# tensorflow/recommenders

Measured on AMD Instinct MI355X. Metric: queries/sec brute-force top-100, higher is better.
Workload: dtype f32; 1 GPU; BruteForce top-100, 1M-item x dim-64 corpus, batch 8192 (BASELINE.json configs[1]); corpus_rows_total=1000000, corpus_rows_per_gpu=1000000, dim=64, batch=8192, k=100, parallelism=single GPU

## Files before the change

include/tfrs_hip.h:

```cpp
#ifndef TFRS_HIP_H_
#define TFRS_HIP_H_

#include <stddef.h>
#include <stdint.h>

#ifdef __cplusplus
extern "C" {
#endif

#define TFRS_OK 0
#define TFRS_EINVAL (-1)
#define TFRS_ENOTIMPL (-2)
#define TFRS_EHIP (-3)
#define TFRS_ENOMEM (-4)
#define TFRS_ESTATE (-5)

#define TFRS_MAX_DIM 128
#define TFRS_MAX_K 1024

int tfrs_version(void);
const char *tfrs_last_error(void);
int tfrs_device_info(int dev, int *cu_count_h, int *lds_bytes_h, char *arch_h,
                     int arch_len);
int tfrs_set_option(const char *name, const char *value);
// ... 37 lines not shown
size_t tfrs_bruteforce_topk_below_workspace_bytes(int64_t nq, int64_t n, int d, int k);
int tfrs_bruteforce_topk_below(const tfrs_index_t *index, const float *queries, int64_t nq, int k,
                               const float *last_scores, const int32_t *last_rows, int64_t last_ld,
                               float *out_scores, int32_t *out_idx, void *workspace,
                               size_t workspace_bytes, void *stream);
int tfrs_bruteforce_topk_redo_count(const void *workspace, int64_t nq, int64_t n, int k,
                                    int32_t *redo_count_h, void *stream);
int tfrs_bruteforce_topk_redo_reasons(const void *workspace, int64_t nq, int64_t n, int k,
                                      int32_t *reasons_h, void *stream);

int tfrs_debug_topk_plan(int64_t n, int k, int shuffled, int64_t *plan_h);

int tfrs_debug_fp16_scores(const tfrs_index_t *index, const float *queries, int64_t nq,
                           int64_t row_begin, int64_t row_end, float *out, float *scratch,
                           void *stream);

size_t tfrs_streaming_topk_workspace_bytes(int64_t nq, int64_t nb, int d, int k);
int tfrs_streaming_topk_update(const float *queries, int64_t nq, int d,
                               const float *cand_block, int64_t nb, int64_t base_row,
                               int k, float *state_scores, int32_t *state_idx,
                               int32_t state_len, int32_t *new_len_h, void *workspace,
                               size_t workspace_bytes, void *stream);

size_t tfrs_streaming_topk_blocks_workspace_bytes(int64_t nq, int64_t total_rows, int d, int k);
int tfrs_streaming_topk_update_blocks(const float *queries, int64_t nq, int d,
                                      const float *const *blocks_h, const int64_t *block_rows_h,
                                      int nblocks, int64_t base_row, int64_t seen_rows, int k,
                                      float *state_scores, int32_t *state_idx, int32_t state_len,
                                      int32_t *new_len_h, void *workspace, size_t workspace_bytes,
                                      void *stream);
// ... 306 lines not shown
```

recommenders_amd/_lib.py:

```python

import ctypes
import os
from typing import Optional

_PKG = os.path.dirname(os.path.abspath(__file__))
LIB_PATH = os.path.join(_PKG, "libtfrs_hip.so")

TFRS_OK, TFRS_EINVAL, TFRS_ENOTIMPL, TFRS_EHIP, TFRS_ENOMEM, TFRS_ESTATE = 0, -1, -2, -3, -4, -5

c_void_p, c_int, c_i64, c_size_t, c_float = (ctypes.c_void_p, ctypes.c_int, ctypes.c_int64,
                                             ctypes.c_size_t, ctypes.c_float)
P = c_void_p
c_u64 = ctypes.c_uint64

SIGNATURES = {
    "tfrs_version": (c_int, []),
    "tfrs_last_error": (ctypes.c_char_p, []),
    "tfrs_device_info": (c_int, [c_int, P, P, P, c_int]),
    "tfrs_set_option": (c_int, [ctypes.c_char_p, ctypes.c_char_p]),
    "tfrs_get_option": (c_int, [ctypes.c_char_p, ctypes.c_char_p, c_int]),
    "tfrs_profile_enable": (c_int, [c_int]),
    "tfrs_profile_read": (c_int, [P, P, P]),
    "tfrs_profile_read_kind": (c_int, [c_int, P, P, P]),
    "tfrs_calibrate_workspace_bytes": (c_size_t, []),
# ... 7 lines not shown
    "tfrs_index_nonfinite": (c_int, [P, c_int, P]),
    "tfrs_index_note_nonfinite": (c_int, [P, P, c_i64, P, c_i64, c_int, P]),
    "tfrs_index_size": (c_i64, [P]),
    "tfrs_index_dim": (c_int, [P]),
    "tfrs_index_unpack": (c_int, [P, P, P]),
    "tfrs_bruteforce_topk_workspace_bytes": (c_size_t, [c_i64, c_i64, c_int, c_int]),
    "tfrs_bruteforce_topk": (c_int, [P, P, c_i64, c_int, P, P, P, c_size_t, P]),
    "tfrs_row_hash64": (c_int, [P, c_i64, c_int, P, P]),
    "tfrs_topk_expand_duplicates": (c_int, [P, P, c_i64, c_int, P, P, c_int, P, P, P]),
    "tfrs_bruteforce_topk_below_workspace_bytes": (c_size_t, [c_i64, c_i64, c_int, c_int]),
    "tfrs_bruteforce_topk_below": (c_int, [P, P, c_i64, c_int, P, P, c_i64, P, P, P, c_size_t, P]),
    "tfrs_bruteforce_topk_redo_count": (c_int, [P, c_i64, c_i64, c_int, P, P]),
    "tfrs_bruteforce_topk_redo_reasons": (c_int, [P, c_i64, c_i64, c_int, P, P]),
    "tfrs_debug_topk_plan": (c_int, [c_i64, c_int, c_int, P]),
    "tfrs_debug_fp16_scores": (c_int, [P, P, c_i64, c_i64, c_i64, P, P, P]),
    "tfrs_streaming_topk_workspace_bytes": (c_size_t, [c_i64, c_i64, c_int, c_int]),
    "tfrs_streaming_topk_update": (c_int, [P, c_i64, c_int, P, c_i64, c_i64, c_int, P, P,
                                           ctypes.c_int32, P, P, c_size_t, P]),
    "tfrs_streaming_topk_blocks_workspace_bytes": (c_size_t, [c_i64, c_i64, c_int, c_int]),
    "tfrs_streaming_topk_update_blocks": (c_int, [P, c_i64, c_int, P, P, c_int, c_i64, c_i64, c_int, P, P,
                                                  ctypes.c_int32, P, P, c_size_t, P]),
    "tfrs_compute_scores": (c_int, [P, P, c_i64, c_int, c_int, P, c_int, P, c_size_t, P]),
    "tfrs_topk_update_from_scores": (c_int, [P, c_i64, c_i64, c_i64, c_i64, c_int, P, P, ctypes.c_int32,
                                             P, P]),
    "tfrs_topk_merge_workspace_bytes": (c_size_t, [c_i64, c_int, c_int, c_int]),
    "tfrs_topk_merge": (c_int, [P, P, c_int, c_i64, c_int, c_int, P, P, P, c_size_t, P]),
    "tfrs_topk_merge_strided": (c_int, [P, P, c_int, c_i64, c_i64, c_int, c_int, P, P, P]),
    "tfrs_topk_exclude": (c_int, [P, P, c_i64, c_int, P, c_int, c_int, P, P, P]),
    "tfrs_rank_of_positive": (c_int, [P, P, c_i64, c_int, P, c_int, P, c_int, P, P]),
    "tfrs_id_match_topk": (c_int, [P, P, c_i64, c_int, P, c_int, P, P]),
# ... 171 lines not shown
```

recommenders_amd/csrc/common.h:

```cpp
#pragma once

#include <hip/hip_runtime.h>
#include <stdint.h>
#include <stdio.h>

#include "../../include/tfrs_hip.h"

namespace tfrs {

void set_error(const char *fmt, ...);

#define TFRS_CHECK_ARG(cond, ...)        \
  do {                                   \
    if (!(cond)) {                       \
      ::tfrs::set_error(__VA_ARGS__);    \
      return TFRS_EINVAL;                \
    }                                    \
  } while (0)

#define TFRS_HIP(call)                                                        \
  do {                                                                        \
    hipError_t e_ = (call);                                                   \
    if (e_ != hipSuccess) {                                                   \
      ::tfrs::set_error("%s failed: %s (%s:%d)", #call, hipGetErrorString(e_), \
// ... 205 lines not shown
  int64_t row_limit;
  int n_qtiles;
  int n_splits;
  const float *lower;
  const float *qk;
  const float *qscale;
  uint32_t *cnt;
  uint2 *buf;
  uint32_t cap_l;
  int nseg;
  float *dense;
  int64_t ld_dense;
  float *binmax;
  int64_t ld_binmax;
  int bin_stages;
  uint32_t *ovf_cnt;
  uint2 *ovf_buf;
  uint32_t ovf_cap;
  int drain_every;
  int drain_min;
  uint32_t *zero_aux;
  uint32_t *zero_word;
};
int launch_scan16(const Scan16Args &a, hipStream_t stream);
constexpr int kScan16QueriesPerWg = 512;

enum SelectSource { kSrcDense = 0, kSrcList = 1, kSrcParts = 2, kSrcRecompute = 3, kSrcExpand = 4 };

struct SelectArgs {
  int64_t nq;
  int k;
  const float *state_scores;
  const int32_t *state_idx;
  int state_len;
  int source;
  const float *dense;
  int64_t ld_dense;
  int64_t n_dense;
  const uint2 *buf;
// ... 61 lines not shown
```

recommenders_amd/csrc/topk_api.hip:

```cpp
#include <stdlib.h>

#include <algorithm>
#include <new>

#include "common.h"

namespace tfrs {

static int64_t env_i64(const char *name, int64_t dflt) {
  const char *v = option(name);
  if (!v || !*v) return dflt;
  return atoll(v);
}

struct TopkTuning {
  int64_t prefix;
  int64_t rho;
  int64_t target_wgs;
  int64_t thr_wgs;
  bool f16_filter;
  int64_t sample;
  int64_t min_bins;
  int64_t drain_min;
  int64_t drain_every;
// ... 392 lines not shown
  se.k = k;
  se.q = q;
  se.d = d;
  se.source = kSrcRecompute;
  se.only_flagged = w.redo;
  se.part_keys = w.part_keys;
  se.idx_base = idx_base;
  se.rc_begin = row_lo;
  se.rc_end = row_lo + n;
  se.raw = raw;
  se.out_scores = out_scores;
  se.out_idx = out_idx;
  return launch_recompute(se, stream);
}

static int run_f16(const float *q, int64_t nq, int d, const char *packed, const F16Image &img,
                   int64_t n, int64_t idx_base, int k, const SamplePlan &sp, bool lower_preset,
                   float *out_scores, int32_t *out_idx, const RoundWs &w, const TopkTuning &t,
                   hipStream_t stream, const int32_t *rowmap = nullptr, int64_t row_lo = 0,
                   const RawTable *raw = nullptr, uint32_t *flags = nullptr) {
  const int n_qtiles = (int)((nq + kScan16QueriesPerWg - 1) / kScan16QueriesPerWg);
  const int64_t stage_lo = row_lo / kTileN;
  int rc;
  if ((rc = launch_query_kappa(q, nq, d, w.qk, w.qscale, w.ovf_cnt, stream, flags)) != TFRS_OK) return rc;

  Scan16Args s16 = {};
  s16.q = q;
  s16.nq = nq;
  s16.d = d;
  s16.packed16 = img.packed16;
  s16.meta = img.meta;
  s16.n_qtiles = n_qtiles;
  s16.qk = w.qk;
  s16.qscale = w.qscale;
  s16.row_limit = row_lo + n;
  s16.stage0 = stage_lo;

  if (!lower_preset) {
  s16.n_stages = (int)sp.n_stages;
  s16.stage_stride = (int)sp.stride;
  {
    TopkTuning tt = t;
    tt.target_wgs = t.thr_wgs;
    plan_stage_splits(sp.n_stages, n_qtiles, tt, &s16.stages_per_split, &s16.n_splits);
  }
  s16.bin_stages = (int)sp.bin_stages;
  s16.stages_per_split = (int)((s16.stages_per_split + sp.bin_stages - 1) / sp.bin_stages * sp.bin_stages);
  s16.n_splits = (int)((sp.n_stages + s16.stages_per_split - 1) / s16.stages_per_split);
  s16.binmax = w.dense;
  s16.ld_binmax = w.ld_dense;
  if ((rc = timed_scan16(s16, 2.0 * (double)nq * (double)sp.n_stages * kTileN * d, stream)) != TFRS_OK)
    return rc;
  if ((rc = launch_bin_threshold(w.dense, w.ld_dense, (int)sp.n_bins(), nq, sp.rank, w.qk,
                                 img.norm_max, w.thr, w.thr_raw, stream)) != TFRS_OK)
    return rc;
  }

  const int64_t all_stages = (n + kTileN - 1) / kTileN;
  s16.binmax = nullptr;
  s16.n_stages = (int)all_stages;
  s16.stage_stride = 1;
  {
    TopkTuning tf = t;
    if (padded_dim16(d) >= 128) tf.target_wgs = std::max<int64_t>(1, t.target_wgs / 2);
    plan_stage_splits(all_stages, n_qtiles, tf, &s16.stages_per_split, &s16.n_splits);
  }
  s16.lower = w.thr;
  s16.cnt = w.cnt;
  s16.buf = w.buf;
  s16.nseg = 2 * s16.n_splits;
  s16.cap_l = segment_cap(k, s16.nseg, t);
// ... 384 lines not shown
  a.packed16 = index->packed16;
  a.meta = index->meta;
  int rc = launch_query_kappa(queries, nq, index->d, scratch, scratch + nq, nullptr, (hipStream_t)stream);
  if (rc != TFRS_OK) return rc;
  a.qk = scratch;
  a.qscale = scratch + nq;
  a.n_qtiles = (int)((nq + kScan16QueriesPerWg - 1) / kScan16QueriesPerWg);
  a.stage0 = row_begin / kTileN;
  a.n_stages = (int)((row_end - row_begin + kTileN - 1) / kTileN);
  a.stage_stride = 1;
  a.row_limit = row_end;
  plan_stage_splits(a.n_stages, a.n_qtiles, t, &a.stages_per_split, &a.n_splits);
  a.dense = out;
  a.ld_dense = (int64_t)a.n_stages * kTileN;
  return launch_scan16(a, (hipStream_t)stream);
}

static bool stream_block_f16(int64_t nb, int k, const TopkTuning &t) {
  return t.f16_filter && k <= kMaxKF16 && nb >= 16 * kTileN;
}
static size_t stream_f16_extra_bytes(int64_t nq, int64_t nb, int d, int k) {
  return align_up((size_t)padded_rows(nb) * row_bytes16(padded_dim16(d))) +
         align_up((size_t)(padded_rows(nb) / kTileN + 1) * sizeof(StageMeta)) +
         2 * align_up((size_t)nq * k * 4);
}

extern "C" size_t tfrs_streaming_topk_workspace_bytes(int64_t nq, int64_t nb, int d, int k) {
  if (nq <= 0 || nb <= 0 || k <= 0 || d <= 0 || d > TFRS_MAX_DIM) return 256;
  const TopkTuning t = tuning();
  size_t b = round_ws_bytes(nq, nb, k, t) + align_up((size_t)padded_rows(nb) * row_bytes(padded_dim(d)));
// ... 625 lines not shown
```

recommenders_amd/csrc/topk_scan16.hip:

```cpp
#include <stdlib.h>

#include <string.h>

#include "common.h"

#ifndef TFRS_SCAN16_ABLATE
#define TFRS_SCAN16_ABLATE 0
#endif
#if TFRS_SCAN16_ABLATE
#ifndef TFRS_ALLOW_ABLATION
#error "TFRS_SCAN16_ABLATE != 0 is a measurement build with wrong results: add -DTFRS_ALLOW_ABLATION to confirm"
#endif
extern "C" int tfrs_ablation_build_scan16(void) { return TFRS_SCAN16_ABLATE; }
#endif
#ifndef TFRS_SCAN16_PEEL
#define TFRS_SCAN16_PEEL 2
#endif

#ifndef TFRS_SCAN16_CLOCKS
#define TFRS_SCAN16_CLOCKS 0
#endif

namespace tfrs {

// ... 91 lines not shown
struct Scan16Mfma {
  static_assert(MF == 32 || (MF == 16 && DP >= 32), "the 16x16x32 shape needs 32 features per instruction");
  static constexpr int kQH = 32 / MF;
  static constexpr int kQW = MF;
  static constexpr int kKPer = 512 / MF;
  static constexpr int kKSteps = DP / kKPer;
  static constexpr int kFrags = DP / 16;
  static constexpr int kChain = kQH * kQH * kKSteps;
  static constexpr int kValuPerMfma = (MF == 16 && DP >= 64) ? 2 : 3;
  static constexpr int a_off(int sub, int m, int row_b) {
    return MF == 32 ? sub * 32 * row_b + m * 32
                    : (sub * 32 + 16 * (m / kKSteps)) * row_b + (m % kKSteps) * 64;
  }
};

template <int DP, int MODE, bool NT = false, int MF = 32>
__global__ void __launch_bounds__(kThreads16, DP <= 64 ? 4 : 2) scan16_kernel(const Scan16Args a) {
  using G = Scan16Geom<DP>;
  using M = Scan16Mfma<DP, MF>;
  static_assert(MF == 32 || MODE != kModeFilter, "the first-generation FILTER exists in the 32x32 shape only");
  constexpr int kNS = kQG * M::kQH;
  extern __shared__ __attribute__((aligned(16))) char smem[];

  const int tid = threadIdx.x;
  const int lane = tid & 63;
  const int wave = __builtin_amdgcn_readfirstlane(tid >> 6);
  if (MODE == kModeFilter && a.zero_word && blockIdx.x == 0 && tid == 0) *a.zero_word = 0u;
  if (MODE == kModeFilter && a.zero_aux && blockIdx.x == 0 && tid < 4) a.zero_aux[tid] = 0u;
  const int j = lane & (MF - 1);
  const int h = lane / MF;

  const int nwg = gridDim.x;
  const int bid = blockIdx.x;
  const int q8 = nwg >> 3, r8 = nwg & 7;
  const int xcd = bid & 7, pos = bid >> 3;
  const int logical = (xcd < r8 ? xcd * (q8 + 1) : r8 * (q8 + 1) + (xcd - r8) * q8) + pos;
  const int split = logical / a.n_qtiles;
  const int qt = logical - split * a.n_qtiles;

  const int i0 = split * a.stages_per_split;
  int i1 = i0 + a.stages_per_split;
  if (i1 > a.n_stages) i1 = a.n_stages;
  if (i0 >= i1) return;
  const int nst = i1 - i0;
  const int64_t stride = a.stage_stride;
  const int64_t first_stage = a.stage0 + (int64_t)i0 * stride;

  f16x8 bq[kNS][M::kKSteps];
  float lower[kNS], qk[kNS], qs[kNS], qinv[kNS];
  bool qvalid[kNS];
  int64_t qrow[kNS];
// ... 97 lines not shown
    float stagemax[kNS];
#pragma unroll
    for (int g = 0; g < kNS; ++g) stagemax[g] = -__builtin_inff();
    const uint32_t stage_row = (uint32_t)((first_stage + (int64_t)st * stride) * kTileN);
    const char *ap = tile + j * G::kRowB + h * 16;

    if (!wave_active) goto stage_done;
    {
    u32x4 af[2][M::kFrags];
#pragma unroll
    for (int m = 0; m < M::kFrags; ++m) af[0][m] = *reinterpret_cast<const u32x4 *>(ap + M::a_off(0, m, G::kRowB));

    f32x16 acc[kQG];
    f32x4 acc4[kNS][2];
    auto chain = [&](int g, int sub) __attribute__((always_inline)) {
      if constexpr (MF == 16) {
#pragma unroll
        for (int qh = 0; qh < 2; ++qh)
#pragma unroll
          for (int ch = 0; ch < 2; ++ch) acc4[2 * g + qh][ch] = f32x4{0.0f, 0.0f, 0.0f, 0.0f};
#pragma unroll
        for (int m = 0; m < M::kKSteps; ++m)
#pragma unroll
          for (int qh = 0; qh < 2; ++qh)
#pragma unroll
            for (int ch = 0; ch < 2; ++ch)
              acc4[2 * g + qh][ch] = __builtin_amdgcn_mfma_f32_16x16x32_f16(
                  as_f16x8(af[sub & 1][ch * M::kKSteps + m]), bq[2 * g + qh][m], acc4[2 * g + qh][ch], 0, 0, 0);
        return;
      }
#pragma unroll
      for (int r = 0; r < 16; ++r) acc[g][r] = 0.0f;
#pragma unroll
      for (int m = 0; m < G::kSteps; ++m)
        acc[g] = __builtin_amdgcn_mfma_f32_32x32x16_f16(as_f16x8(af[sub & 1][m]), bq[g][m], acc[g], 0, 0, 0);
    };
    auto check = [&](int g, int sub) __attribute__((always_inline)) {
      if constexpr (MF == 16) {
#pragma unroll
        for (int qh = 0; qh < 2; ++qh) {
          const int s = 2 * g + qh;
          if (MODE == kModeMaterialize) {
            if (qvalid[s]) {
              float *drow = a.dense + qrow[s] * a.ld_dense + ((int64_t)(i0 + st) * kTileN + sub * 32 + 4 * h);
#pragma unroll
              for (int ch = 0; ch < 2; ++ch)
                *reinterpret_cast<float4 *>(drow + 16 * ch) =
                    make_float4(acc4[s][ch][0] * unscale[s], acc4[s][ch][1] * unscale[s],
                                acc4[s][ch][2] * unscale[s], acc4[s][ch][3] * unscale[s]);
            }
          } else {
            stagemax[s] = __builtin_fmaxf(stagemax[s], max8(acc4[s][0], acc4[s][1]));
            asm volatile("" : "+v"(stagemax[s]));
          }
        }
        return;
      }
      const f32x16 &c = acc[g];
      if (MODE == kModeMaterialize) {
        if (qvalid[g]) {
          float *drow = a.dense + qrow[g] * a.ld_dense +
                        ((int64_t)(i0 + st) * kTileN + sub * 32 + 4 * h);
#pragma unroll
          for (int g4 = 0; g4 < 4; ++g4)
            *reinterpret_cast<float4 *>(drow + 8 * g4) =
                make_float4(c[4 * g4 + 0] * unscale[g], c[4 * g4 + 1] * unscale[g],
                            c[4 * g4 + 2] * unscale[g], c[4 * g4 + 3] * unscale[g]);
        }
        return;
      }
      const float m0 = max16(c);
      if (MODE == kModeBinMax) {
        stagemax[g] = __builtin_fmaxf(stagemax[g], m0);
        asm volatile("" : "+v"(stagemax[g]));
        return;
      }
      if (__ballot(m0 > thr[g]) != 0ull) {
        const uint32_t rbase = stage_row + sub * 32 + 4u * h;
#pragma unroll
        for (int g4 = 0; g4 < 4; ++g4) {
          const float gm = __builtin_fmaxf(mx3(c[4 * g4], c[4 * g4 + 1], c[4 * g4 + 2]), c[4 * g4 + 3]);
          if (__ballot(gm > thr[g]) == 0ull) continue;
#pragma unroll
          for (int rr = 0; rr < 4; ++rr) {
            const float v = c[4 * g4 + rr];
            const uint32_t row = rbase + rr + 8 * g4;
            if (v > thr[g] && row < row_limit) {
              if (mycnt[g] < a.cap_l) *wp[g] = make_uint2(__float_as_uint(v * unscale[g]), row);
              wp[g] += a.nseg;
              ++mycnt[g];
            }
// ... 49 lines not shown
        }
      }
    }
    wait_dma();
    __syncthreads();
  }

  if (MODE == kModeFilter) {
#pragma unroll
    for (int g = 0; g < kNS; ++g)
      if (qvalid[g]) a.cnt[qrow[g] * a.nseg + 2 * split + h] = mycnt[g];
  }
}


template <int DP, int NW, int QG, int SPB = 1, int MF = 32>
struct Scan16FGeom : Scan16Geom<DP> {
  using B = Scan16Geom<DP>;
  static constexpr int kTiles = NW * QG * 32 / kScan16QueriesPerWg;
  static constexpr int kWavesPerTile = NW / kTiles;
  static_assert(kTiles >= 1 && kTiles * kScan16QueriesPerWg == NW * QG * 32, "queries per workgroup");
  static constexpr int kThreads = NW * 64;
  static constexpr int kLoadsF = (B::kChunks + kThreads - 1) / kThreads;
  static constexpr int kQCap = 32;
  static constexpr int kEntB = MF == 16 ? 48 : 80;
  static constexpr int kWaveB = kQCap * kEntB + QG * 64 * 4 + QG * 64 * 16;
  static constexpr int kSlots = 2 * SPB;
  static constexpr int kMetaOffF = kSlots * B::kStageB;
  static constexpr int kQueueOff = (kMetaOffF + kSlots * 16 + 15) / 16 * 16;
  static constexpr int kLdsBytesF = kQueueOff + NW * kWaveB;
  static_assert(kLdsBytesF <= 160 * 1024, "LDS budget");
};

template <int CHUNKS, int LOADS, int THREADS, bool NT = false>
__device__ __forceinline__ void stage16f_glds(const char *gsrc, char *lds_dst, const StageMeta *meta,
                                              char *lds_meta, int tid, int wave) {
#pragma unroll
  for (int i = 0; i < LOADS; ++i) {
    const int ch0 = i * THREADS + wave * 64;
    if (ch0 < CHUNKS)
      glds_copy16<NT>(gsrc + (size_t)(i * THREADS + tid) * 16, lds_dst + ch0 * 16);
  }
  if (tid == 0) glds_copy16(reinterpret_cast<const char *>(meta), lds_meta);
}
// ... 11 lines not shown
  constexpr int kNS = QG * M::kQH;
  extern __shared__ __attribute__((aligned(16))) char smem[];

  const int tid = threadIdx.x;
  const int lane = tid & 63;
  const int wave = __builtin_amdgcn_readfirstlane(tid >> 6);
  if (a.zero_word && blockIdx.x == 0 && tid == 0) *a.zero_word = 0u;
  if (a.zero_aux && blockIdx.x == 0 && tid < 4) a.zero_aux[tid] = 0u;
  long long clk0 = 0, wall0 = 0;
  if (TFRS_SCAN16_CLOCKS) { clk0 = clock64(); wall0 = wall_clock64(); }
  const int j = lane & (MF - 1);
  const int h = lane / MF;
  const int tj = lane & 31;
  const int th = lane >> 5;

  const int nwg = gridDim.x;
  const int bid = blockIdx.x;
  const int q8 = nwg >> 3, r8 = nwg & 7;
  const int xcd = bid & 7, pos = bid >> 3;
  const int logical = (xcd < r8 ? xcd * (q8 + 1) : r8 * (q8 + 1) + (xcd - r8) * q8) + pos;
  const int n_qgroups = (a.n_qtiles + G::kTiles - 1) / G::kTiles;
  const int split = logical / n_qgroups;
  const int qt = (logical - split * n_qgroups) * G::kTiles + wave / G::kWavesPerTile;
  const int wave_in_tile = wave % G::kWavesPerTile;

  const int i0 = split * a.stages_per_split;
  int i1 = i0 + a.stages_per_split;
  if (i1 > a.n_stages) i1 = a.n_stages;
  if (i0 >= i1) return;
  const int nst = i1 - i0;
  const int64_t first_stage = a.stage0 + (int64_t)i0 * a.stage_stride;

  char *const qbase = smem + G::kQueueOff + wave * G::kWaveB;
  uint32_t *const wcnt = reinterpret_cast<uint32_t *>(qbase + G::kQCap * G::kEntB);
  #pragma unroll
// ... 166 lines not shown
    for (int s = 0; s < kNS; ++s) {
      const float4 qc = qconst[MF == 16 ? (s >> 1) * 64 + (s & 1) * 16 + j : s * 64 + lane];
      thr[s] = __builtin_fmaf(-qc.y, s_norm, qc.x) * s_inv;
    }
    const uint32_t stage_row = (uint32_t)((first_stage + (int64_t)st * a.stage_stride) * kTileN);
    const char *ap = tile + j * G::kRowB + h * 16;

    u32x4 af[2][M::kFrags];
#pragma unroll
    for (int m = 0; m < M::kFrags; ++m) af[0][m] = *reinterpret_cast<const u32x4 *>(ap + M::a_off(0, m, G::kRowB));

    f32x16 acc[QG];
    f32x4 acc4[kNS][2];
    if (TFRS_SCAN16_ABLATE & 32) __builtin_amdgcn_s_setprio(2);
    auto chain = [&](int g, int sub) __attribute__((always_inline)) {
      if constexpr (MF == 16) {
#pragma unroll
        for (int qh = 0; qh < 2; ++qh)
#pragma unroll
          for (int ch = 0; ch < 2; ++ch) acc4[2 * g + qh][ch] = f32x4{0.0f, 0.0f, 0.0f, 0.0f};
#pragma unroll
        for (int m = 0; m < M::kKSteps; ++m)
#pragma unroll
          for (int qh = 0; qh < 2; ++qh)
#pragma unroll
            for (int ch = 0; ch < 2; ++ch)
              acc4[2 * g + qh][ch] = __builtin_amdgcn_mfma_f32_16x16x32_f16(
                  as_f16x8(af[sub & 1][ch * M::kKSteps + m]), bq[2 * g + qh][m], acc4[2 * g + qh][ch], 0, 0, 0);
        return;
      }
#pragma unroll
      for (int r = 0; r < 16; ++r) acc[g][r] = 0.0f;
#pragma unroll
      for (int m = 0; m < G::kSteps; ++m)
        acc[g] = __builtin_amdgcn_mfma_f32_32x32x16_f16(as_f16x8(af[sub & 1][m]), bq[g][m], acc[g], 0, 0, 0);
    };
    auto check16 = [&](int g, int sub) __attribute__((always_inline)) {
      f32x4 (&c)[kNS][2] = acc4;
      if (TFRS_SCAN16_PEEL == 2)
        asm volatile("s_nop 7" : "+v"(c[2 * g][0]), "+v"(c[2 * g][1]), "+v"(c[2 * g + 1][0]), "+v"(c[2 * g + 1][1]));
      if (TFRS_SCAN16_ABLATE & 16) { asm volatile("" :: "v"(c[2 * g][0][0]), "v"(c[2 * g + 1][1][3])); return; }
      bool hot[2];
      uint64_t hm[2];
#pragma unroll
      for (int qh = 0; qh < 2; ++qh) {
        hot[qh] = max8(c[2 * g + qh][0], c[2 * g + qh][1]) > thr[2 * g + qh];
        hm[qh] = __ballot(hot[qh]);
      }
      if (TFRS_SCAN16_ABLATE & 2) { asm volatile("" :: "s"(hm[0]), "s"(hm[1])); return; }
      if (__builtin_expect((hm[0] | hm[1]) != 0ull, 0)) {
// ... 158 lines not shown
  __builtin_amdgcn_wave_barrier();
  int ln = lane;
  asm volatile("" : "+v"(ln));
#pragma unroll
  for (int g = 0; g < QG; ++g) {
    const int64_t qrow = q0 + g * 32 + (ln & 31);
    if (qrow < a.nq) a.cnt[qrow * a.nseg + 2 * split + (ln >> 5)] = wcnt[g * 64 + ln];
  }
#if TFRS_SCAN16_CLOCKS
  if (blockIdx.x == 0 && tid == 0)
    printf("scan16f_clocks mfma %d dim %d cycles %lld ticks100MHz %lld\n", MF, DP, clock64() - clk0, wall_clock64() - wall0);
#endif
}


static bool scan16_nt_copies(const Scan16Args &a) {
  const char *e = option("TFRS_SCAN16_NT");
  return a.n_qtiles == 1 && !(e && e[0] == '0');
}

template <int DP>
constexpr bool kScan16Has16x16 = DP >= 32 && TFRS_SCAN16_PEEL != 1;
constexpr int scan16_default_mfma(int dp) { return dp >= 64 ? 16 : 32; }

static int scan16_mfma(int dp, int *mf) {
  const char *e = option("TFRS_SCAN16_MFMA");
  *mf = scan16_default_mfma(dp);
  if (e) {
    if (strcmp(e, "32x32") == 0) *mf = 32;
    else if (strcmp(e, "16x16") == 0) *mf = 16;
// ... 46 lines not shown
}

template <int DP, int MODE, bool NT = false, int MF = 32>
static int launch_scan16_variant(const Scan16Args &a, hipStream_t stream) {
  using G = Scan16Geom<DP>;
  if constexpr (MODE == kModeBinMax && !NT) {
    if (scan16_nt_copies(a)) return launch_scan16_variant<DP, MODE, true, MF>(a, stream);
  }
  TFRS_HIP(ensure_dynamic_lds(reinterpret_cast<const void *>(&scan16_kernel<DP, MODE, NT, MF>), G::kLdsBytes));
  const dim3 grid((unsigned)(a.n_qtiles * a.n_splits));
  hipLaunchKernelGGL((scan16_kernel<DP, MODE, NT, MF>), grid, dim3(kThreads16), G::kLdsBytes, stream, a);
  TFRS_LAUNCH_CHECK();
  return TFRS_OK;
}

template <int DP>
static int launch_scan16_dp(const Scan16Args &a, hipStream_t stream) {
  if (a.dense || a.binmax) {
    int mf;
    if (const int rc = scan16_mfma(DP, &mf)) return rc;
    if constexpr (kScan16Has16x16<DP>) {
      if (mf == 16)
        return a.dense ? launch_scan16_variant<DP, kModeMaterialize, false, 16>(a, stream)
                       : launch_scan16_variant<DP, kModeBinMax, false, 16>(a, stream);
    }
    return a.dense ? launch_scan16_variant<DP, kModeMaterialize>(a, stream)
                   : launch_scan16_variant<DP, kModeBinMax>(a, stream);
  }
  return launch_scan16_variant<DP, kModeFilter>(a, stream);
}

static int scan16_generation() {
  const char *e = option("TFRS_SCAN16_V");
  return (e && e[0] == '1') ? 1 : 2;
}

int launch_scan16(const Scan16Args &a_in, hipStream_t stream) {
  Scan16Args a = a_in;
  if (a.nq <= 0 || a.n_stages <= 0) return TFRS_OK;
  if (a.drain_min < 1) a.drain_min = 1;
  if (a.drain_every < 1) a.drain_every = 1;
  TFRS_CHECK_ARG(a.stage_stride >= 1 && a.stages_per_split >= 1 &&
                     (int64_t)a.n_splits * a.stages_per_split >= a.n_stages,
                 "scan16: bad stage split");
  TFRS_CHECK_ARG(a.dense || a.binmax || a.nseg == 2 * a.n_splits, "scan16: nseg must be 2 * n_splits");
  TFRS_CHECK_ARG(!a.binmax || (a.bin_stages >= 1 && a.stages_per_split % a.bin_stages == 0),
                 "scan16: stages_per_split must be a multiple of bin_stages");
  const bool fits32 = (uint64_t)a.nq * a.cap_l * (uint64_t)a.nseg < (1ull << 32);
  if (!a.dense && !a.binmax && fits32 && scan16_generation() == 2) {
    switch (padded_dim16(a.d)) {
      case 16: return launch_scan16f_shape<16>(a, stream);
      case 32: return launch_scan16f_shape<32>(a, stream);
      case 64: return launch_scan16f_shape<64>(a, stream);
      case 128: return launch_scan16f_shape<128>(a, stream);
    }
  }
  switch (padded_dim16(a.d)) {
    case 16: return launch_scan16_dp<16>(a, stream);
    case 32: return launch_scan16_dp<32>(a, stream);
    case 64: return launch_scan16_dp<64>(a, stream);
    case 128: return launch_scan16_dp<128>(a, stream);
  }
// ... 6 lines not shown
```

Baseline: 8.166 million queries/s.

## Add 16-wave wide bin-max threshold kernel sharing staged corpus tiles across query tiles

Adds a dedicated 16-wave binmax kernel for the threshold (sampling) pass that processes two query tiles per workgroup. Staged fp16 corpus tiles are shared across more queries and loaded with a multi-stage double buffer (SPB=4). This is meant to cut LDS staging traffic and global reads per query in the threshold pass. It is selected automatically when the query-tile count is even and at least 16 with dim up to 64, so at batch 8192 (16 tiles) it is used. The change also factors the MFMA chain, tile-max and XCD remap into shared helpers and adds a debug entry point; the bigger workgroups risk lower occupancy and fewer splits.

```diff
diff --git a/include/tfrs_hip.h b/include/tfrs_hip.h
--- a/include/tfrs_hip.h
+++ b/include/tfrs_hip.h
@@ -75,6 +75,10 @@
 int tfrs_debug_fp16_scores(const tfrs_index_t *index, const float *queries, int64_t nq,
                            int64_t row_begin, int64_t row_end, float *out, float *scratch,
                            void *stream);
+
+int tfrs_debug_threshold_pass(const tfrs_index_t *index, const float *queries, int64_t nq, int k,
+                              float *lower, float *thr_raw, int32_t *applicable_h, void *workspace,
+                              size_t workspace_bytes, void *stream);
 
 size_t tfrs_streaming_topk_workspace_bytes(int64_t nq, int64_t nb, int d, int k);
 int tfrs_streaming_topk_update(const float *queries, int64_t nq, int d,
diff --git a/recommenders_amd/_lib.py b/recommenders_amd/_lib.py
--- a/recommenders_amd/_lib.py
+++ b/recommenders_amd/_lib.py
@@ -45,6 +45,7 @@
     "tfrs_bruteforce_topk_redo_reasons": (c_int, [P, c_i64, c_i64, c_int, P, P]),
     "tfrs_debug_topk_plan": (c_int, [c_i64, c_int, c_int, P]),
     "tfrs_debug_fp16_scores": (c_int, [P, P, c_i64, c_i64, c_i64, P, P, P]),
+    "tfrs_debug_threshold_pass": (c_int, [P, P, c_i64, c_int, P, P, P, P, c_size_t, P]),
     "tfrs_streaming_topk_workspace_bytes": (c_size_t, [c_i64, c_i64, c_int, c_int]),
     "tfrs_streaming_topk_update": (c_int, [P, c_i64, c_int, P, c_i64, c_i64, c_int, P, P,
                                            ctypes.c_int32, P, P, c_size_t, P]),
diff --git a/recommenders_amd/csrc/common.h b/recommenders_amd/csrc/common.h
--- a/recommenders_amd/csrc/common.h
+++ b/recommenders_amd/csrc/common.h
@@ -243,6 +243,7 @@
   float *binmax;
   int64_t ld_binmax;
   int bin_stages;
+  int thr_wide;
   uint32_t *ovf_cnt;
   uint2 *ovf_buf;
   uint32_t ovf_cap;
@@ -252,6 +253,7 @@
   uint32_t *zero_word;
 };
 int launch_scan16(const Scan16Args &a, hipStream_t stream);
+int scan16_threshold_form(int n_qtiles, int d, int *wide);
 constexpr int kScan16QueriesPerWg = 512;
 
 enum SelectSource { kSrcDense = 0, kSrcList = 1, kSrcParts = 2, kSrcRecompute = 3, kSrcExpand = 4 };
diff --git a/recommenders_amd/csrc/topk_api.hip b/recommenders_amd/csrc/topk_api.hip
--- a/recommenders_amd/csrc/topk_api.hip
+++ b/recommenders_amd/csrc/topk_api.hip
@@ -430,6 +430,33 @@
   return launch_recompute(se, stream);
 }
 
+static int run_f16_threshold(Scan16Args &s16, int64_t nq, int d, const SamplePlan &sp, const F16Image &img,
+                             const RoundWs &w, const TopkTuning &t, hipStream_t stream) {
+  int rc;
+  s16.n_stages = (int)sp.n_stages;
+  s16.stage_stride = (int)sp.stride;
+  if ((rc = scan16_threshold_form(s16.n_qtiles, d, &s16.thr_wide)) != TFRS_OK) return rc;
+  {
+    TopkTuning tt = t;
+    tt.target_wgs = t.thr_wgs;
+    int wgs_per_split = s16.n_qtiles;
+    if (s16.thr_wide) {
+      tt.target_wgs = std::max<int64_t>(1, t.thr_wgs / 2);
+      wgs_per_split = (s16.n_qtiles + 1) / 2;
+    }
+    plan_stage_splits(sp.n_stages, wgs_per_split, tt, &s16.stages_per_split, &s16.n_splits);
+  }
+  s16.bin_stages = (int)sp.bin_stages;
+  s16.stages_per_split = (int)((s16.stages_per_split + sp.bin_stages - 1) / sp.bin_stages * sp.bin_stages);
+  s16.n_splits = (int)((sp.n_stages + s16.stages_per_split - 1) / s16.stages_per_split);
+  s16.binmax = w.dense;
+  s16.ld_binmax = w.ld_dense;
+  if ((rc = timed_scan16(s16, 2.0 * (double)nq * (double)sp.n_stages * kTileN * d, stream)) != TFRS_OK)
+    return rc;
+  return launch_bin_threshold(w.dense, w.ld_dense, (int)sp.n_bins(), nq, sp.rank, w.qk, img.norm_max, w.thr,
+                              w.thr_raw, stream);
+}
+
 static int run_f16(const float *q, int64_t nq, int d, const char *packed, const F16Image &img,
                    int64_t n, int64_t idx_base, int k, const SamplePlan &sp, bool lower_preset,
                    float *out_scores, int32_t *out_idx, const RoundWs &w, const TopkTuning &t,
@@ -452,25 +479,8 @@
   s16.row_limit = row_lo + n;
   s16.stage0 = stage_lo;
 
-  if (!lower_preset) {
-  s16.n_stages = (int)sp.n_stages;
-  s16.stage_stride = (int)sp.stride;
-  {
-    TopkTuning tt = t;
-    tt.target_wgs = t.thr_wgs;
-    plan_stage_splits(sp.n_stages, n_qtiles, tt, &s16.stages_per_split, &s16.n_splits);
-  }
-  s16.bin_stages = (int)sp.bin_stages;
-  s16.stages_per_split = (int)((s16.stages_per_split + sp.bin_stages - 1) / sp.bin_stages * sp.bin_stages);
-  s16.n_splits = (int)((sp.n_stages + s16.stages_per_split - 1) / s16.stages_per_split);
-  s16.binmax = w.dense;
-  s16.ld_binmax = w.ld_dense;
-  if ((rc = timed_scan16(s16, 2.0 * (double)nq * (double)sp.n_stages * kTileN * d, stream)) != TFRS_OK)
-    return rc;
-  if ((rc = launch_bin_threshold(w.dense, w.ld_dense, (int)sp.n_bins(), nq, sp.rank, w.qk,
-                                 img.norm_max, w.thr, w.thr_raw, stream)) != TFRS_OK)
-    return rc;
-  }
+  if (!lower_preset && (rc = run_f16_threshold(s16, nq, d, sp, img, w, t, stream)) != TFRS_OK) return rc;
+  s16.thr_wide = 0;
 
   const int64_t all_stages = (n + kTileN - 1) / kTileN;
   s16.binmax = nullptr;
@@ -885,6 +895,48 @@
   a.dense = out;
   a.ld_dense = (int64_t)a.n_stages * kTileN;
   return launch_scan16(a, (hipStream_t)stream);
+}
+
+extern "C" int tfrs_debug_threshold_pass(const tfrs_index_t *index, const float *queries, int64_t nq, int k,
+                                         float *lower, float *thr_raw, int32_t *applicable_h, void *workspace,
+                                         size_t workspace_bytes, void *stream) {
+  if (!index || !index->packed16) {
+    set_error("debug_threshold_pass: the index has not been built");
+    return TFRS_ESTATE;
+  }
+  TFRS_CHECK_ARG(queries && lower && thr_raw && applicable_h && workspace && nq > 0,
+                 "debug_threshold_pass: bad argument");
+  TFRS_CHECK_ARG(k >= 1 && k <= TFRS_MAX_K && (int64_t)k <= index->n, "debug_threshold_pass: k=%d out of range", k);
+  const TopkTuning t = tuning();
+  *applicable_h = 0;
+  if (!(t.f16_filter && k <= kMaxKF16)) return TFRS_OK;
+  const SamplePlan sp = plan_sample(index->n, k, t, use_stat(t, index->rowmap));
+  if (sp.n_stages <= 0) return TFRS_OK;
+  const size_t need = round_ws_bytes(nq, index->n, k, t);
+  if (workspace_bytes < need) {
+    set_error("debug_threshold_pass: workspace %zu < required %zu", workspace_bytes, need);
+    return TFRS_ENOMEM;
+  }
+  const RoundWs w = carve_round_ws(static_cast<char *>(workspace), nq, index->n, k, t);
+  const F16Image img = {index->packed16, index->meta, index->norm_max};
+  int rc = launch_query_kappa(queries, nq, index->d, w.qk, w.qscale, w.ovf_cnt, (hipStream_t)stream);
+  if (rc != TFRS_OK) return rc;
+  Scan16Args s16 = {};
+  s16.q = queries;
+  s16.nq = nq;
+  s16.d = index->d;
+  s16.packed16 = img.packed16;
+  s16.meta = img.meta;
+  s16.n_qtiles = (int)((nq + kScan16QueriesPerWg - 1) / kScan16QueriesPerWg);
+  s16.qk = w.qk;
+  s16.qscale = w.qscale;
+  s16.row_limit = index->n;
+  s16.stage0 = 0;
+  if ((rc = run_f16_threshold(s16, nq, index->d, sp, img, w, t, (hipStream_t)stream)) != TFRS_OK) return rc;
+  TFRS_HIP(hipMemcpyAsync(lower, w.thr, (size_t)nq * 4, hipMemcpyDeviceToDevice, (hipStream_t)stream));
+  TFRS_HIP(hipMemcpyAsync(thr_raw, w.thr_raw, (size_t)nq * 4, hipMemcpyDeviceToDevice, (hipStream_t)stream));
+  *applicable_h = 1;
+  return TFRS_OK;
 }
 
 static bool stream_block_f16(int64_t nb, int k, const TopkTuning &t) {
diff --git a/recommenders_amd/csrc/topk_scan16.hip b/recommenders_amd/csrc/topk_scan16.hip
--- a/recommenders_amd/csrc/topk_scan16.hip
+++ b/recommenders_amd/csrc/topk_scan16.hip
@@ -129,6 +129,72 @@
   }
 };
 
+__device__ __forceinline__ int scan16_logical_wg() {
+  const int nwg = gridDim.x;
+  const int bid = blockIdx.x;
+  const int q8 = nwg >> 3, r8 = nwg & 7;
+  const int xcd = bid & 7, pos = bid >> 3;
+  return (xcd < r8 ? xcd * (q8 + 1) : r8 * (q8 + 1) + (xcd - r8) * q8) + pos;
+}
+
+template <int DP, int MF, int NS>
+__device__ __forceinline__ void scan16_chain(int g, const u32x4 (&af)[Scan16Mfma<DP, MF>::kFrags],
+                                             const f16x8 (&bq)[NS][Scan16Mfma<DP, MF>::kKSteps],
+                                             f32x16 (&acc)[NS / Scan16Mfma<DP, MF>::kQH], f32x4 (&acc4)[NS][2]) {
+  using M = Scan16Mfma<DP, MF>;
+  if constexpr (MF == 16) {
+#pragma unroll
+    for (int qh = 0; qh < 2; ++qh)
+#pragma unroll
+      for (int ch = 0; ch < 2; ++ch) acc4[2 * g + qh][ch] = f32x4{0.0f, 0.0f, 0.0f, 0.0f};
+#pragma unroll
+    for (int m = 0; m < M::kKSteps; ++m)
+#pragma unroll
+      for (int qh = 0; qh < 2; ++qh)
+#pragma unroll
+        for (int ch = 0; ch < 2; ++ch)
+          acc4[2 * g + qh][ch] = __builtin_amdgcn_mfma_f32_16x16x32_f16(
+              as_f16x8(af[ch * M::kKSteps + m]), bq[2 * g + qh][m], acc4[2 * g + qh][ch], 0, 0, 0);
+  } else {
+#pragma unroll
+    for (int r = 0; r < 16; ++r) acc[g][r] = 0.0f;
+#pragma unroll
+    for (int m = 0; m < DP / 16; ++m)
+      acc[g] = __builtin_amdgcn_mfma_f32_32x32x16_f16(as_f16x8(af[m]), bq[g][m], acc[g], 0, 0, 0);
+  }
+}
+
+template <int MF, int NS>
+__device__ __forceinline__ void scan16_tile_max(int g, const f32x16 (&acc)[NS * MF / 32], const f32x4 (&acc4)[NS][2],
+                                                float (&stagemax)[NS]) {
+  if constexpr (MF == 16) {
+#pragma unroll
+    for (int qh = 0; qh < 2; ++qh) {
+      const int s = 2 * g + qh;
+      stagemax[s] = __builtin_fmaxf(stagemax[s], max8(acc4[s][0], acc4[s][1]));
+      asm volatile("" : "+v"(stagemax[s]));
+    }
+  } else {
+    stagemax[g] = __builtin_fmaxf(stagemax[g], max16(acc[g]));
+    asm volatile("" : "+v"(stagemax[g]));
+  }
+}
+
+template <int MF, int NS>
+__device__ __forceinline__ void scan16_store_bin(const Scan16Args &a, int64_t q0, int j, int h, int bin,
+                                                 const float (&binmax)[NS]) {
+#pragma unroll
+  for (int s = 0; s < NS; ++s) {
+    const int64_t qrow = q0 + s * MF + j;
+    if constexpr (MF == 16) {
+      const float v = __builtin_fmaxf(binmax[s], __shfl_xor(binmax[s], 16));
+      if (qrow < a.nq && (h & 1) == 0) a.binmax[qrow * a.ld_binmax + 2 * bin + (h >> 1)] = v;
+    } else {
+      if (qrow < a.nq) a.binmax[qrow * a.ld_binmax + 2 * bin + h] = binmax[s];
+    }
+  }
+}
+
 template <int DP, int MODE, bool NT = false, int MF = 32>
 __global__ void __launch_bounds__(kThreads16, DP <= 64 ? 4 : 2) scan16_kernel(const Scan16Args a) {
   using G = Scan16Geom<DP>;
@@ -145,11 +211,7 @@
   const int j = lane & (MF - 1);
   const int h = lane / MF;
 
-  const int nwg = gridDim.x;
-  const int bid = blockIdx.x;
-  const int q8 = nwg >> 3, r8 = nwg & 7;
-  const int xcd = bid & 7, pos = bid >> 3;
-  const int logical = (xcd < r8 ? xcd * (q8 + 1) : r8 * (q8 + 1) + (xcd - r8) * q8) + pos;
+  const int logical = scan16_logical_wg();
   const int split = logical / a.n_qtiles;
   const int qt = logical - split * a.n_qtiles;
 
@@ -277,44 +339,24 @@
     f32x16 acc[kQG];
     f32x4 acc4[kNS][2];
     auto chain = [&](int g, int sub) __attribute__((always_inline)) {
-      if constexpr (MF == 16) {
-#pragma unroll
-        for (int qh = 0; qh < 2; ++qh)
-#pragma unroll
-          for (int ch = 0; ch < 2; ++ch) acc4[2 * g + qh][ch] = f32x4{0.0f, 0.0f, 0.0f, 0.0f};
-#pragma unroll
-        for (int m = 0; m < M::kKSteps; ++m)
-#pragma unroll
-          for (int qh = 0; qh < 2; ++qh)
-#pragma unroll
-            for (int ch = 0; ch < 2; ++ch)
-              acc4[2 * g + qh][ch] = __builtin_amdgcn_mfma_f32_16x16x32_f16(
-                  as_f16x8(af[sub & 1][ch * M::kKSteps + m]), bq[2 * g + qh][m], acc4[2 * g + qh][ch], 0, 0, 0);
-        return;
-      }
-#pragma unroll
-      for (int r = 0; r < 16; ++r) acc[g][r] = 0.0f;
-#pragma unroll
-      for (int m = 0; m < G::kSteps; ++m)
-        acc[g] = __builtin_amdgcn_mfma_f32_32x32x16_f16(as_f16x8(af[sub & 1][m]), bq[g][m], acc[g], 0, 0, 0);
+      scan16_chain<DP, MF, kNS>(g, af[sub & 1], bq, acc, acc4);
     };
     auto check = [&](int g, int sub) __attribute__((always_inline)) {
+      if constexpr (MODE == kModeBinMax) {
+        scan16_tile_max<MF, kNS>(g, acc, acc4, stagemax);
+        return;
+      }
       if constexpr (MF == 16) {
 #pragma unroll
         for (int qh = 0; qh < 2; ++qh) {
           const int s = 2 * g + qh;
-          if (MODE == kModeMaterialize) {
-            if (qvalid[s]) {
-              float *drow = a.dense + qrow[s] * a.ld_dense + ((int64_t)(i0 + st) * kTileN + sub * 32 + 4 * h);
-#pragma unroll
-              for (int ch = 0; ch < 2; ++ch)
-                *reinterpret_cast<float4 *>(drow + 16 * ch) =
-                    make_float4(acc4[s][ch][0] * unscale[s], acc4[s][ch][1] * unscale[s],
-                                acc4[s][ch][2] * unscale[s], acc4[s][ch][3] * unscale[s]);
-            }
-          } else {
-            stagemax[s] = __builtin_fmaxf(stagemax[s], max8(acc4[s][0], acc4[s][1]));
-            asm volatile("" : "+v"(stagemax[s]));
+          if (qvalid[s]) {
+            float *drow = a.dense + qrow[s] * a.ld_dense + ((int64_t)(i0 + st) * kTileN + sub * 32 + 4 * h);
+#pragma unroll
+            for (int ch = 0; ch < 2; ++ch)
+              *reinterpret_cast<float4 *>(drow + 16 * ch) =
+                  make_float4(acc4[s][ch][0] * unscale[s], acc4[s][ch][1] * unscale[s],
+                              acc4[s][ch][2] * unscale[s], acc4[s][ch][3] * unscale[s]);
           }
         }
         return;
@@ -333,11 +375,6 @@
         return;
       }
       const float m0 = max16(c);
-      if (MODE == kModeBinMax) {
-        stagemax[g] = __builtin_fmaxf(stagemax[g], m0);
-        asm volatile("" : "+v"(stagemax[g]));
-        return;
-      }
       if (__ballot(m0 > thr[g]) != 0ull) {
         const uint32_t rbase = stage_row + sub * 32 + 4u * h;
 #pragma unroll
@@ -417,20 +454,27 @@
 }
 
 
-template <int DP, int NW, int QG, int SPB = 1, int MF = 32>
-struct Scan16FGeom : Scan16Geom<DP> {
+template <int DP, int NW, int QG, int SPB>
+struct Scan16WideGeom : Scan16Geom<DP> {
   using B = Scan16Geom<DP>;
   static constexpr int kTiles = NW * QG * 32 / kScan16QueriesPerWg;
   static constexpr int kWavesPerTile = NW / kTiles;
   static_assert(kTiles >= 1 && kTiles * kScan16QueriesPerWg == NW * QG * 32, "queries per workgroup");
   static constexpr int kThreads = NW * 64;
   static constexpr int kLoadsF = (B::kChunks + kThreads - 1) / kThreads;
+  static constexpr int kSlots = 2 * SPB;
+  static constexpr int kMetaOffF = kSlots * B::kStageB;
+  static constexpr int kStagesEnd = kMetaOffF + kSlots * 16;
+  static_assert(kStagesEnd <= 160 * 1024, "LDS budget");
+};
+
+template <int DP, int NW, int QG, int SPB = 1, int MF = 32>
+struct Scan16FGeom : Scan16WideGeom<DP, NW, QG, SPB> {
+  using W = Scan16WideGeom<DP, NW, QG, SPB>;
   static constexpr int kQCap = 32;
   static constexpr int kEntB = MF == 16 ? 48 : 80;
   static constexpr int kWaveB = kQCap * kEntB + QG * 64 * 4 + QG * 64 * 16;
-  static constexpr int kSlots = 2 * SPB;
-  static constexpr int kMetaOffF = kSlots * B::kStageB;
-  static constexpr int kQueueOff = (kMetaOffF + kSlots * 16 + 15) / 16 * 16;
+  static constexpr int kQueueOff = (W::kStagesEnd + 15) / 16 * 16;
   static constexpr int kLdsBytesF = kQueueOff + NW * kWaveB;
   static_assert(kLdsBytesF <= 160 * 1024, "LDS budget");
 };
@@ -472,11 +516,7 @@
   const int tj = lane & 31;
   const int th = lane >> 5;
 
-  const int nwg = gridDim.x;
-  const int bid = blockIdx.x;
-  const int q8 = nwg >> 3, r8 = nwg & 7;
-  const int xcd = bid & 7, pos = bid >> 3;
-  const int logical = (xcd < r8 ? xcd * (q8 + 1) : r8 * (q8 + 1) + (xcd - r8) * q8) + pos;
+  const int logical = scan16_logical_wg();
   const int n_qgroups = (a.n_qtiles + G::kTiles - 1) / G::kTiles;
   const int split = logical / n_qgroups;
   const int qt = (logical - split * n_qgroups) * G::kTiles + wave / G::kWavesPerTile;
@@ -673,26 +713,7 @@
     f32x4 acc4[kNS][2];
     if (TFRS_SCAN16_ABLATE & 32) __builtin_amdgcn_s_setprio(2);
     auto chain = [&](int g, int sub) __attribute__((always_inline)) {
-      if constexpr (MF == 16) {
-#pragma unroll
-        for (int qh = 0; qh < 2; ++qh)
-#pragma unroll
-          for (int ch = 0; ch < 2; ++ch) acc4[2 * g + qh][ch] = f32x4{0.0f, 0.0f, 0.0f, 0.0f};
-#pragma unroll
-        for (int m = 0; m < M::kKSteps; ++m)
-#pragma unroll
-          for (int qh = 0; qh < 2; ++qh)
-#pragma unroll
-            for (int ch = 0; ch < 2; ++ch)
-              acc4[2 * g + qh][ch] = __builtin_amdgcn_mfma_f32_16x16x32_f16(
-                  as_f16x8(af[sub & 1][ch * M::kKSteps + m]), bq[2 * g + qh][m], acc4[2 * g + qh][ch], 0, 0, 0);
-        return;
-      }
-#pragma unroll
-      for (int r = 0; r < 16; ++r) acc[g][r] = 0.0f;
-#pragma unroll
-      for (int m = 0; m < G::kSteps; ++m)
-        acc[g] = __builtin_amdgcn_mfma_f32_32x32x16_f16(as_f16x8(af[sub & 1][m]), bq[g][m], acc[g], 0, 0, 0);
+      scan16_chain<DP, MF, kNS>(g, af[sub & 1], bq, acc, acc4);
     };
     auto check16 = [&](int g, int sub) __attribute__((always_inline)) {
       f32x4 (&c)[kNS][2] = acc4;
@@ -881,6 +902,191 @@
 }
 
 
+
+template <int DP, int MF, int NS>
+__device__ __forceinline__ void scan16_query_operands(const Scan16Args &a, int64_t q0, int j, int h,
+                                                      f16x8 (&bq)[NS][Scan16Mfma<DP, MF>::kKSteps], float (&qs)[NS]) {
+  using M = Scan16Mfma<DP, MF>;
+  const bool vec_ok = (a.d == DP) && ((reinterpret_cast<uintptr_t>(a.q) & 15) == 0);
+  float4 qlo[NS][M::kKSteps], qhi[NS][M::kKSteps];
+#pragma unroll
+  for (int s = 0; s < NS; ++s) {
+    const int64_t qrow = q0 + s * M::kQW + j;
+    qs[s] = a.qscale[qrow < a.nq ? qrow : a.nq - 1];
+  }
+  if (vec_ok) {
+#pragma unroll
+    for (int s = 0; s < NS; ++s) {
+      const int64_t qrow = q0 + s * M::kQW + j;
+      const float *qp = a.q + (qrow < a.nq ? qrow : a.nq - 1) * a.d;
+#pragma unroll
+      for (int m = 0; m < M::kKSteps; ++m) {
+        qlo[s][m] = *reinterpret_cast<const float4 *>(qp + M::kKPer * m + 8 * h);
+        qhi[s][m] = *reinterpret_cast<const float4 *>(qp + M::kKPer * m + 8 * h + 4);
+      }
+    }
+  }
+#pragma unroll
+  for (int s = 0; s < NS; ++s) {
+    const int64_t qrow = q0 + s * M::kQW + j;
+    const bool qvalid = qrow < a.nq;
+    const float *qp = a.q + (qvalid ? qrow : a.nq - 1) * a.d;
+    if (!qvalid) qs[s] = 1.0f;
+    const float qinv = 1.0f / qs[s];
+#pragma unroll
+    for (int m = 0; m < M::kKSteps; ++m) {
+      float x[8];
+      if (vec_ok) {
+        float4 lo = qlo[s][m], hi = qhi[s][m];
+        if (!qvalid) lo = hi = make_float4(0.f, 0.f, 0.f, 0.f);
+        x[0] = lo.x; x[1] = lo.y; x[2] = lo.z; x[3] = lo.w;
+        x[4] = hi.x; x[5] = hi.y; x[6] = hi.z; x[7] = hi.w;
+      } else {
+#pragma unroll
+        for (int i = 0; i < 8; ++i) {
+          const int k = M::kKPer * m + 8 * h + i;
+          x[i] = (qvalid && k < a.d) ? qp[k] : 0.0f;
+        }
+      }
+      u32x4 w;
+#pragma unroll
+      for (int i = 0; i < 4; ++i) w[i] = cvt_f16x2(x[2 * i] * qinv, x[2 * i + 1] * qinv);
+      bq[s][m] = as_f16x8(w);
+    }
+  }
+}
+
+template <int DP, int MF, int SPB>
+__global__ void __launch_bounds__(16 * 64) binmax16w_kernel(const Scan16Args a) {
+  using G = Scan16WideGeom<DP, 16, kQG, SPB>;
+  using M = Scan16Mfma<DP, MF>;
+  constexpr int kNS = kQG * M::kQH;
+  extern __shared__ __attribute__((aligned(16))) char smem[];
+
+  const int tid = threadIdx.x;
+  const int lane = tid & 63;
+  const int wave = __builtin_amdgcn_readfirstlane(tid >> 6);
+  const int j = lane & (MF - 1);
+  const int h = lane / MF;
+
+  const int logical = scan16_logical_wg();
+  const int n_qgroups = (a.n_qtiles + G::kTiles - 1) / G::kTiles;
+  const int split = logical / n_qgroups;
+  const int qt = (logical - split * n_qgroups) * G::kTiles + wave / G::kWavesPerTile;
+  const int wave_in_tile = wave % G::kWavesPerTile;
+
+  const int i0 = split * a.stages_per_split;
+  int i1 = i0 + a.stages_per_split;
+  if (i1 > a.n_stages) i1 = a.n_stages;
+  if (i0 >= i1) return;
+  const int nst = i1 - i0;
+  const int64_t first_stage = a.stage0 + (int64_t)i0 * a.stage_stride;
+
+  static_assert(G::kChunks % 64 == 0, "stage size must be a whole number of wave copies");
+  const char *gsrc = a.packed16 + first_stage * (int64_t)G::kStageB;
+  const int64_t gstep = (int64_t)a.stage_stride * (int64_t)G::kStageB;
+  const StageMeta *mp = a.meta + first_stage;
+  auto copy_stage = [&](int st) __attribute__((always_inline)) {
+    const int slot = ((st / SPB) & 1) * SPB + (st % SPB);
+    stage16f_glds<G::kChunks, G::kLoadsF, G::kThreads>(gsrc + (int64_t)st * gstep, smem + slot * G::kStageB,
+                                                      mp + (int64_t)st * a.stage_stride,
+                                                      smem + G::kMetaOffF + slot * 16, tid, wave);
+  };
+#pragma unroll
+  for (int u = 0; u < SPB; ++u)
+    if (u < nst) copy_stage(u);
+
+  const int64_t q0 = (int64_t)qt * kScan16QueriesPerWg + wave_in_tile * (kQG * 32);
+  const bool wave_active = q0 < a.nq;
+  f16x8 bq[kNS][M::kKSteps];
+  float qs[kNS];
+  scan16_query_operands<DP, MF, kNS>(a, q0, j, h, bq, qs);
+  wait_dma();
+  __syncthreads();
+
+  float binmax[kNS];
+#pragma unroll
+  for (int s = 0; s < kNS; ++s) binmax[s] = -__builtin_inff();
+  int bin = i0 / a.bin_stages;
+  int bin_fill = 0;
+
+  const int n_periods = (nst + SPB - 1) / SPB;
+  for (int per = 0; per < n_periods; ++per) {
+#pragma unroll
+    for (int u = 0; u < SPB; ++u)
+      if ((per + 1) * SPB + u < nst) copy_stage((per + 1) * SPB + u);
+#pragma unroll
+    for (int u = 0; u < SPB; ++u) {
+      const int st = per * SPB + u;
+      if (st >= nst) break;
+      if (!wave_active) continue;
+      const int slot = (per & 1) * SPB + u;
+      const char *tile = smem + slot * G::kStageB;
+      const StageMeta sm = *reinterpret_cast<const StageMeta *>(smem + G::kMetaOffF + slot * 16);
+      const float s_scale = __uint_as_float(__builtin_amdgcn_readfirstlane(__float_as_uint(sm.scale)));
+      float stagemax[kNS];
+#pragma unroll
+      for (int s = 0; s < kNS; ++s) stagemax[s] = -__builtin_inff();
+      const char *ap = tile + j * G::kRowB + h * 16;
+
+      u32x4 af[2][M::kFrags];
+#pragma unroll
+      for (int m = 0; m < M::kFrags; ++m) af[0][m] = *reinterpret_cast<const u32x4 *>(ap + M::a_off(0, m, G::kRowB));
+      f32x16 acc[kQG];
+      f32x4 acc4[kNS][2];
+      auto chain = [&](int g, int sub) __attribute__((always_inline)) {
+        scan16_chain<DP, MF, kNS>(g, af[sub & 1], bq, acc, acc4);
+      };
+      auto check = [&](int g) __attribute__((always_inline)) {
+        if constexpr (MF == 16)
+          asm volatile("s_nop 7" : "+v"(acc4[2 * g][0]), "+v"(acc4[2 * g][1]), "+v"(acc4[2 * g + 1][0]), "+v"(acc4[2 * g + 1][1]));
+        else
+          asm volatile("s_nop 11" : "+v"(acc[g]));
+        scan16_tile_max<MF, kNS>(g, acc, acc4, stagemax);
+      };
+      auto interleave = [&]() __attribute__((always_inline)) {
+#pragma unroll
+        for (int i = 0; i < M::kChain; ++i) {
+          __builtin_amdgcn_sched_group_barrier(0x008, 1, 0);
+          __builtin_amdgcn_sched_group_barrier(0x002, M::kValuPerMfma, 0);
+        }
+      };
+      chain(0, 0);
+#pragma unroll
+      for (int sub = 0; sub < kTileN / 32; ++sub) {
+        if (sub + 1 < kTileN / 32) {
+#pragma unroll
+          for (int m = 0; m < M::kFrags; ++m)
+            af[(sub + 1) & 1][m] = *reinterpret_cast<const u32x4 *>(ap + M::a_off(sub + 1, m, G::kRowB));
+        }
+        __builtin_amdgcn_sched_barrier(0);
+        chain(1, sub);
+        check(0);
+        interleave();
+        if (sub + 1 < kTileN / 32) {
+          chain(0, sub + 1);
+          check(1);
+          interleave();
+        } else {
+          check(1);
+        }
+      }
+#pragma unroll
+      for (int s = 0; s < kNS; ++s) binmax[s] = __builtin_fmaxf(binmax[s], stagemax[s] * (qs[s] * s_scale));
+      if (++bin_fill == a.bin_stages || st == nst - 1) {
+        scan16_store_bin<MF, kNS>(a, q0, j, h, bin, binmax);
+        ++bin;
+        bin_fill = 0;
+#pragma unroll
+        for (int s = 0; s < kNS; ++s) binmax[s] = -__builtin_inff();
+      }
+    }
+    wait_dma();
+    __syncthreads();
+  }
+}
+
+
 static bool scan16_nt_copies(const Scan16Args &a) {
   const char *e = option("TFRS_SCAN16_NT");
   return a.n_qtiles == 1 && !(e && e[0] == '0');
@@ -957,11 +1163,43 @@
   return TFRS_OK;
 }
 
+template <int DP, int MF, int SPB>
+static int launch_binmax16w(const Scan16Args &a, hipStream_t stream) {
+  using G = Scan16WideGeom<DP, 16, kQG, SPB>;
+  TFRS_HIP(ensure_dynamic_lds(reinterpret_cast<const void *>(&binmax16w_kernel<DP, MF, SPB>), G::kStagesEnd));
+  const dim3 grid((unsigned)((a.n_qtiles + G::kTiles - 1) / G::kTiles * a.n_splits));
+  hipLaunchKernelGGL((binmax16w_kernel<DP, MF, SPB>), grid, dim3(G::kThreads), G::kStagesEnd, stream, a);
+  TFRS_LAUNCH_CHECK();
+  return TFRS_OK;
+}
+
+constexpr int kThrSpb = 4;
+constexpr int kThrWideMinTiles = 16;
+int scan16_threshold_form(int n_qtiles, int d, int *wide) {
+  const char *e = option("TFRS_SCAN16_THR");
+  const bool classic = e && strcmp(e, "classic") == 0;
+  if (e && !classic && strcmp(e, "wide") != 0) {
+    set_error("TFRS_SCAN16_THR=%s: expected wide or classic", e);
+    return TFRS_EINVAL;
+  }
+  const bool exists = n_qtiles >= 2 && padded_dim16(d) <= 64;
+  *wide = (exists && !classic && (e || (n_qtiles % 2 == 0 && n_qtiles >= kThrWideMinTiles))) ? 1 : 0;
+  return TFRS_OK;
+}
+
 template <int DP>
 static int launch_scan16_dp(const Scan16Args &a, hipStream_t stream) {
   if (a.dense || a.binmax) {
     int mf;
     if (const int rc = scan16_mfma(DP, &mf)) return rc;
+    if constexpr (DP <= 64) {
+      if (a.binmax && a.thr_wide) {
+        if constexpr (kScan16Has16x16<DP>) {
+          if (mf == 16) return launch_binmax16w<DP, 16, kThrSpb>(a, stream);
+        }
+        return launch_binmax16w<DP, 32, kThrSpb>(a, stream);
+      }
+    }
     if constexpr (kScan16Has16x16<DP>) {
       if (mf == 16)
         return a.dense ? launch_scan16_variant<DP, kModeMaterialize, false, 16>(a, stream)
@@ -989,6 +1227,8 @@
   TFRS_CHECK_ARG(a.dense || a.binmax || a.nseg == 2 * a.n_splits, "scan16: nseg must be 2 * n_splits");
   TFRS_CHECK_ARG(!a.binmax || (a.bin_stages >= 1 && a.stages_per_split % a.bin_stages == 0),
                  "scan16: stages_per_split must be a multiple of bin_stages");
+  TFRS_CHECK_ARG(!a.thr_wide || (a.binmax && padded_dim16(a.d) <= 64),
+                 "scan16: the 16-wave threshold kernel exists up to dim 64");
   const bool fits32 = (uint64_t)a.nq * a.cap_l * (uint64_t)a.nseg < (1ull << 32);
   if (!a.dense && !a.binmax && fits32 && scan16_generation() == 2) {
     switch (padded_dim16(a.d)) {
```

After: 8.204 million queries/s, median of 6. About the same (+0.5%).
